# sail-sg/finetune-fair-diffusion

Measured on AMD Instinct MI355X. Metric: training-images/sec (SD-v1.5 512^2, 20-step DPM-Solver++ unroll, fairness-finetune step), higher is better.
Workload: dtype f16

## Files before the change

finetune_fair_diffusion_amd/csrc/gemm.hip:

```cpp
#include "gemm_device.h"

template <int BM, int BN, bool CONV>
__global__ __launch_bounds__(256) void gemm_glds_kernel(fd_gemm_desc p, int ntm, int ntn) {
    FD_WG_TRACE(1);
    constexpr int TM = BM / 32, TN = BN / 32;
    constexpr int AI = BM / 64, BI = BN / 64;
    constexpr int EPI_HALFS = 4 * (BM / 2) * (BN / 2 + 4);
    constexpr int OPS_HALFS = 2 * (BM + BN) * 32;
    __shared__ __attribute__((aligned(16))) f16 smem[OPS_HALFS > EPI_HALFS ? OPS_HALFS : EPI_HALFS];
    f16* As = smem;
    f16* Bs = smem + 2 * BM * 32;
    const f16* zp = fd_zero_page;
    asm volatile("" : "+s"(zp));

    const int tid = threadIdx.x, lane = tid & 63, wave = tid >> 6;
    const int l15 = lane & 15, lg = lane >> 4;
    const int wm = wave >> 1, wn = wave & 1;

    const int tile = xcd_remap(blockIdx.x, ntm * ntn);
    const int m0 = (tile / ntn) * BM, n0 = (tile % ntn) * BN;
    const int z = blockIdx.y;

    const f16* A = (const f16*)p.A + (int64_t)z * p.sA;
    const f16* B = (const f16*)p.B + (int64_t)z * p.sB;
// ... 448 lines not shown
    const int ntm = (d.M + BM - 1) / BM, ntn = (d.N + BN - 1) / BN;
    constexpr size_t lds = (size_t)2 * (BM + BN) * 64 * sizeof(f16);
    static std::once_flag once;
    std::call_once(once, [] {
        (void)hipFuncSetAttribute((const void*)gemm_big_kernel<BM, BN, WGM, WGN, 0>, hipFuncAttributeMaxDynamicSharedMemorySize, (int)lds);
        (void)hipFuncSetAttribute((const void*)gemm_big_kernel<BM, BN, WGM, WGN, 1>, hipFuncAttributeMaxDynamicSharedMemorySize, (int)lds);
        (void)hipFuncSetAttribute((const void*)gemm_big_kernel<BM, BN, WGM, WGN, 2>, hipFuncAttributeMaxDynamicSharedMemorySize, (int)lds);
    });
    static const long l2_budget = bench_env("FD_GEMM_L2_KB") ? atol(bench_env("FD_GEMM_L2_KB")) * 1024 : 3 * 1024 * 1024;
    const long ktot = ((long)d.K + d.K2) / nsplit;
    const int nph = (d.conv && (d.conv_mode == FD_CONV_UP2P || d.conv_mode == FD_CONV_UP2PI)) ? 4 : 1;
    long gnl = l2_budget / ((long)BN * ktot * 2);
    const int gn = (int)(gnl < 1 ? 1 : (gnl > ntn ? ntn : gnl));
    if constexpr (BN / WGN == 80) {
        if (d.gn_stats && nsplit == 1 && d.conv && d.conv_mode == FD_CONV_UP2PI) {
            static std::once_flag once_st6;
            std::call_once(once_st6, [] {
                (void)hipFuncSetAttribute((const void*)gemm_big_kernel<BM, BN, WGM, WGN, 6>, hipFuncAttributeMaxDynamicSharedMemorySize, (int)lds);
            });
            hipLaunchKernelGGL((gemm_big_kernel<BM, BN, WGM, WGN, 6>), dim3(ntm * ntn * nph, 1), dim3(WGM * WGN * 64), lds, s, d, ntm, ntn, gn);
            return fd_check_launch("fd_gemm(big, phase pair with statistics epilogue)");
        }
        if (d.gn_stats && nsplit == 1 && !(d.conv && d.conv_mode >= FD_CONV_UP2P)) {
            static std::once_flag once_st;
            std::call_once(once_st, [] {
                (void)hipFuncSetAttribute((const void*)gemm_big_kernel<BM, BN, WGM, WGN, 3>, hipFuncAttributeMaxDynamicSharedMemorySize, (int)lds);
                (void)hipFuncSetAttribute((const void*)gemm_big_kernel<BM, BN, WGM, WGN, 4>, hipFuncAttributeMaxDynamicSharedMemorySize, (int)lds);
            });
            if (d.conv) hipLaunchKernelGGL((gemm_big_kernel<BM, BN, WGM, WGN, 4>), dim3(ntm * ntn, 1), dim3(WGM * WGN * 64), lds, s, d, ntm, ntn, gn);
            else hipLaunchKernelGGL((gemm_big_kernel<BM, BN, WGM, WGN, 3>), dim3(ntm * ntn, 1), dim3(WGM * WGN * 64), lds, s, d, ntm, ntn, gn);
            return fd_check_launch("fd_gemm(big, statistics epilogue)");
        }
    }
    if (d.conv && d.conv_mode >= FD_CONV_UP2P)
        hipLaunchKernelGGL((gemm_big_kernel<BM, BN, WGM, WGN, 2>), dim3(ntm * ntn * nph, nsplit), dim3(WGM * WGN * 64), lds, s, d, ntm, ntn, gn);
    else if (d.conv) hipLaunchKernelGGL((gemm_big_kernel<BM, BN, WGM, WGN, 1>), dim3(ntm * ntn, nsplit), dim3(WGM * WGN * 64), lds, s, d, ntm, ntn, gn);
    else hipLaunchKernelGGL((gemm_big_kernel<BM, BN, WGM, WGN, 0>), dim3(ntm * ntn, nsplit), dim3(WGM * WGN * 64), lds, s, d, ntm, ntn, gn);
    if (nsplit > 1) return launch_splitk_reduce(d, s, nsplit);
    return fd_check_launch("fd_gemm(big)");
}


template <int NT, int KS, int RT>
__global__ __launch_bounds__(KS * 64) void gemm_skinny_kernel(fd_gemm_desc p) {
    FD_WG_TRACE(4);
    __shared__ float red[KS > 1 ? (KS - 1) * RT * NT * 256 : 1];
    const int lane = threadIdx.x & 63, wave = threadIdx.x >> 6;
    const int l15 = lane & 15, lg = lane >> 4;
    const f16* A[RT];
    bool mok[RT];
#pragma unroll
    for (int r = 0; r < RT; ++r) {
        const int m = (blockIdx.x * RT + r) * 16 + l15;
        mok[r] = m < p.M;
        A[r] = (const f16*)p.A + (int64_t)(mok[r] ? m : 0) * p.lda + lg * 8;
    }
    const f16* B = (const f16*)p.B + lg * 8;
    f32x4 acc[RT][NT];
#pragma unroll
    for (int r = 0; r < RT; ++r)
#pragma unroll
        for (int j = 0; j < NT; ++j) acc[r][j] = (f32x4){0.f, 0.f, 0.f, 0.f};
    const int nks = p.K >> 5;
    const int per = (nks + KS - 1) / KS;
    const int kbeg = wave * per, kend = min(nks, kbeg + per);
    constexpr int CH = 10 / RT;
    for (int k0 = kbeg; k0 < kend; k0 += CH) {
        f16x8 af[RT][CH];
#pragma unroll
        for (int c = 0; c < CH; ++c)
#pragma unroll
            for (int r = 0; r < RT; ++r) {
                af[r][c] = (f16x8){0, 0, 0, 0, 0, 0, 0, 0};
                if (k0 + c < kend && mok[r]) af[r][c] = *(const f16x8*)(A[r] + (int64_t)(k0 + c) * 32);
            }
#pragma unroll
        for (int c = 0; c < CH; ++c) {
            if (k0 + c < kend) {
#pragma unroll
                for (int j = 0; j < NT; ++j) {
                    const int n = j * 16 + l15;
                    f16x8 bf = (f16x8){0, 0, 0, 0, 0, 0, 0, 0};
                    if (n < p.N) bf = *(const f16x8*)(B + (int64_t)n * p.ldb + (int64_t)(k0 + c) * 32);
#pragma unroll
                    for (int r = 0; r < RT; ++r) acc[r][j] = FD_MFMA_16x16x32(bf, af[r][c], acc[r][j]);
                }
            }
        }
    }
    if (KS > 1) {
        if (wave > 0) {
#pragma unroll
            for (int r = 0; r < RT; ++r)
#pragma unroll
                for (int j = 0; j < NT; ++j) *(f32x4*)(red + ((((wave - 1) * RT + r) * NT + j) * 64 + lane) * 4) = acc[r][j];
        }
        __syncthreads();
        if (wave > 0) return;
#pragma unroll
        for (int w = 1; w < KS; ++w)
#pragma unroll
            for (int r = 0; r < RT; ++r)
#pragma unroll
                for (int j = 0; j < NT; ++j) acc[r][j] += *(const f32x4*)(red + ((((w - 1) * RT + r) * NT + j) * 64 + lane) * 4);
    }
#pragma unroll
    for (int r = 0; r < RT; ++r) {
        if (!mok[r]) continue;
        f16* C = (f16*)p.C + (int64_t)((blockIdx.x * RT + r) * 16 + l15) * p.ldc;
#pragma unroll
        for (int j = 0; j < NT; ++j) {
            const int n = j * 16 + lg * 4;
            if (n < p.N) *(f16x4*)(C + n) = (f16x4){(f16)acc[r][j][0], (f16)acc[r][j][1], (f16)acc[r][j][2], (f16)acc[r][j][3]};
        }
    }
}

static bool skinny_ok(const fd_gemm_desc& d) {
    static const bool off = bench_env("FD_GEMM_NOSKINNY") != nullptr;
    if (d.N > 16 && d.M >= 32768) return false;
    return !off && !d.conv && d.batch <= 1 && d.K2 == 0 && d.colscale_cols == 0 && d.N <= 64 && (d.N & 3) == 0 && (d.K & 31) == 0 && d.M >= 1024 && !d.bias && !d.rowbias &&
           !d.residual && d.act == FD_ACT_NONE && d.alpha == 1.f && d.out_dtype == FD_OUT_F16 && (d.ldc & 3) == 0;
}

template <int NT, int RT>
static int launch_skinny_rt(const fd_gemm_desc& d, hipStream_t s) {
    const int blocks = (d.M + 16 * RT - 1) / (16 * RT);
    const int ks = d.K >= 1280 ? 4 : d.K >= 640 ? 2 : 1;
    if (ks == 4) hipLaunchKernelGGL((gemm_skinny_kernel<NT, 4, RT>), dim3(blocks), dim3(256), 0, s, d);
    else if (ks == 2) hipLaunchKernelGGL((gemm_skinny_kernel<NT, 2, RT>), dim3(blocks), dim3(128), 0, s, d);
    else hipLaunchKernelGGL((gemm_skinny_kernel<NT, 1, RT>), dim3(blocks), dim3(64), 0, s, d);
    return fd_check_launch("fd_gemm(skinny)");
}

template <int NT>
static int launch_skinny(const fd_gemm_desc& d, hipStream_t s) {
    static const int rt = bench_env("FD_GEMM_SKINNY_RT") ? atoi(bench_env("FD_GEMM_SKINNY_RT")) : 0;
    const bool two = rt == 2;
    return two ? launch_skinny_rt<NT, 2>(d, s) : launch_skinny_rt<NT, 1>(d, s);
}

template <int BM, int BN>
static int launch(const fd_gemm_desc& d, hipStream_t s) {
    const int ntm = (d.M + BM - 1) / BM, ntn = (d.N + BN - 1) / BN;
    dim3 grid(ntm * ntn, d.batch > 0 ? d.batch : 1);
    if (d.conv) hipLaunchKernelGGL((gemm_glds_kernel<BM, BN, true>), grid, dim3(256), 0, s, d, ntm, ntn);
    else hipLaunchKernelGGL((gemm_glds_kernel<BM, BN, false>), grid, dim3(256), 0, s, d, ntm, ntn);
    return fd_check_launch("fd_gemm");
}

bool fd_gemm_pp_eligible(const fd_gemm_desc& d);
int fd_gemm_launch_pp(const fd_gemm_desc& d, hipStream_t s, bool prio, int bm, int nsplit);
bool fd_conv_halo_takes(const fd_gemm_desc& d, int bm, int nsplit);
#ifndef FD_GEMM_PP_DEFAULT
#define FD_GEMM_PP_DEFAULT (1 | 4 | 8 | 32)
#endif
static int pp_mode() {
#ifdef FD_BENCH_HOOKS
    const char* e = getenv("FD_GEMM_PP");
    return e ? atoi(e) : FD_GEMM_PP_DEFAULT;
#else
    return FD_GEMM_PP_DEFAULT;
#endif
}
static int pp_takes(const fd_gemm_desc& d, int sel) {
    const int t = sel % 1000000, split = sel / 1000000, m = pp_mode();
    if (!m || !fd_gemm_pp_eligible(d)) return 0;
    if (t == 256320 && split == 0) {
        if (d.conv) return (m & 1) ? 256 : 0;
        if ((m & 2) || ((m & 32) && d.K + d.K2 <= 384 && d.N >= 2560)) return 256;
        return 0;
    }
    if (t == 128320 && (split == 0 || (m & 64))) return (m & (d.conv ? 8 : 16)) ? 128 : 0;
    return 0;
}

static int gemm_tile(const fd_gemm_desc& d);
extern "C" int fd_gemm_tile(const fd_gemm_desc* dp) {
    FD_REQUIRE_DESC(dp, fd_gemm_desc, "fd_gemm_tile");
    return gemm_tile(*dp);
}
static int gemm_tile(const fd_gemm_desc& d) {
    const long nb = d.batch > 1 ? d.batch : 1;
    static const bool nobig = bench_env("FD_GEMM_NOBIG") != nullptr;
    static const int force = bench_env("FD_GEMM_FORCE") ? atoi(bench_env("FD_GEMM_FORCE")) : 0;
    if (skinny_ok(d)) return 16000 + (d.N + 15) / 16 * 16;
    if (force && nb == 1 && !d.conv) return force;
    static const int bigk = bench_env("FD_GEMM_BIGK") ? atoi(bench_env("FD_GEMM_BIGK")) : 320;
    if (!nobig && nb == 1 && (d.conv ? (d.Cin & 63) == 0 : (d.K + d.K2) >= bigk)) {
        const long phs = (d.conv && (d.conv_mode == FD_CONV_UP2P || d.conv_mode == FD_CONV_UP2PI)) ? 4 : 1;
        const long m256 = phs * ((d.M + 255) / 256), m128 = phs * ((d.M + 127) / 128);
        static const long t256 = bench_env("FD_GEMM_T256") ? atol(bench_env("FD_GEMM_T256")) : 100;
        static const long t128 = bench_env("FD_GEMM_T128") ? atol(bench_env("FD_GEMM_T128")) : 80;
        static const long maxsplit = bench_env("FD_GEMM_MAXSPLIT") ? atol(bench_env("FD_GEMM_MAXSPLIT")) : 8;
        static const long tc256 = bench_env("FD_CONV_T256") ? atol(bench_env("FD_CONV_T256")) : 0;
        if (d.N % 320 == 0) {
            if (m256 * (d.N / 320) >= ((tc256 && d.conv && d.conv_mode == FD_CONV_NORMAL) ? tc256 : t256)) return 256320;
            if (m128 * (d.N / 320) >= t128) return 128320;
        }
        const bool can_split = d.workspace && (d.N & 3) == 0 && (d.ldc & 3) == 0 && d.act != FD_ACT_GEGLU && phs == 1;
        const long nk = (d.K + 63) / 64 + (d.K2 + 63) / 64;
        auto split_for = [&](long blocks, int tilecode) -> int {
            long split = blocks > 0 ? 256 / blocks : 1;
            if (split > maxsplit) split = maxsplit;
            while (split > 1 && (nk / split < 8 || (int64_t)split * d.M * d.N * 4 > d.workspace_bytes)) --split;
            return split > 1 ? (int)(split * 1000000 + tilecode) : 0;
        };
        if (can_split && nk >= 64 && d.N % 320 == 0 && m128 * (d.N / 320) >= 32) {
            const int c = split_for(m128 * (d.N / 320), 128320);
            if (c) return c;
        }
        static const long t160 = bench_env("FD_GEMM_T160") ? atol(bench_env("FD_GEMM_T160")) : 160;
        if (d.N % 160 == 0 && m128 * (d.N / 160) >= t160) return 128160;
        static const bool no256 = bench_env("FD_GEMM_NO256256") != nullptr;
        static const long tvae = bench_env("FD_GEMM_TVAE") ? atol(bench_env("FD_GEMM_TVAE")) : 200;
        if (!no256 && d.N % 256 == 0 && m256 * (d.N / 256) >= tvae) return 256256;
        static const bool no512 = bench_env("FD_GEMM_NO512128") != nullptr;
        if (!no512 && d.N == 128 && ((d.M + 511) / 512) >= 400) return 512128;
        if (d.N % 128 == 0 && m256 * (d.N / 128) >= tvae) return 256128;
        if (can_split && d.N % 160 == 0) {
            const int c = split_for(m128 * (d.N / 160), 128160);
            if (c) return c;
        }
    }
    const long t128 = (long)((d.M + 127) / 128) * ((d.N + 127) / 128) * nb;
    const bool n64 = (d.N % 128) != 0 && (d.N % 128) <= 64;
    if (t128 >= 512 && !n64) return 128128;
    const long t12864 = (long)((d.M + 127) / 128) * ((d.N + 63) / 64) * nb;
    if (t12864 >= 512) return 128064;
    return 64064;
}

enum { GK_SKINNY, GK_GLDS, GK_BIG, GK_PP };
struct GemmPlan { int kind, bm, bn, wgm, wgn, nsplit, cv; bool stats_ok; };
static GemmPlan gemm_plan(const fd_gemm_desc& d ) {
    GemmPlan g = {};
    const int sel = gemm_tile(d), t = sel % 1000000;
    static const bool w16 = bench_env("FD_GEMM_W8") == nullptr;
    g.nsplit = sel >= 1000000 ? sel / 1000000 : 1;
    g.bm = t / 1000; g.bn = t % 1000;
    g.cv = d.conv ? (d.conv_mode >= FD_CONV_UP2P ? 2 : 1) : 0;
    if (const int bm = pp_takes(d, sel)) { g.kind = GK_PP; g.bm = bm; g.bn = 320; g.wgm = 2; g.wgn = 4; }
    else if (g.nsplit > 1) { g.kind = GK_BIG; g.wgm = 4; g.wgn = t == 128320 ? 4 : 2; }
    else switch (t) {
        case 256320: g.kind = GK_BIG; g.wgm = (w16 && !d.conv) ? 4 : 2; g.wgn = 4; break;
        case 128320: g.kind = GK_BIG; g.wgm = w16 ? 4 : 2; g.wgn = 4; break;
        case 128160: g.kind = GK_BIG; g.wgm = 4; g.wgn = 2; break;
        case 256256: g.kind = GK_BIG; g.wgm = 2; g.wgn = 4; break;
        case 512128: g.kind = GK_BIG; g.wgm = 8; g.wgn = 2; break;
        case 256128: g.kind = GK_BIG; g.wgm = 4; g.wgn = 2; break;
        default: g.kind = g.bm == 16 ? GK_SKINNY : GK_GLDS; break;
    }
    const bool lds_epi = d.out_dtype == FD_OUT_F16 && (d.N & 7) == 0 && (d.ldc & 7) == 0 && (!d.residual || (d.ldr & 7) == 0) &&
                         (!d.rowbias || (d.ld_rowbias & 3) == 0);
    g.stats_ok = (g.kind == GK_PP || (g.kind == GK_BIG && g.bn / g.wgn == 80)) && g.nsplit == 1 && lds_epi && d.act != FD_ACT_GEGLU &&
                 d.batch <= 1 && (d.N % 80) == 0 && (g.cv < 2 || (d.conv_mode == FD_CONV_UP2PI && (d.M & 31) == 0));
    return g;
}

extern "C" int fd_gemm_kernel_name(const fd_gemm_desc* dp, char* buf, int n) {
    FD_REQUIRE_DESC(dp, fd_gemm_desc, "fd_gemm_kernel_name");
    fd_gemm_desc d = *dp;
    if (d.K2 <= 0 || !d.A2) d.K2 = 0;
    const GemmPlan g = gemm_plan(d);
    const bool st = d.gn_stats && g.stats_ok;
    switch (g.kind) {
        case GK_PP:
            if (fd_conv_halo_takes(d, g.bm, g.nsplit)) snprintf(buf, n, "conv_halo_kernel<%d, %d, %d, %s>", g.bm, d.W, st ? 3 : 1, (pp_mode() & 4) ? "true" : "false");
            else snprintf(buf, n, "gemm_pp_kernel<%d, %d, %s>", g.bm, (d.conv ? 1 : 0) + (st ? 2 : 0), (pp_mode() & 4) ? "true" : "false");
            break;
        case GK_BIG: snprintf(buf, n, "gemm_big_kernel<%d, %d, %d, %d, %d>", g.bm, g.bn, g.wgm, g.wgn, st ? (g.cv == 2 ? 6 : g.cv + 3) : g.cv); break;
        case GK_SKINNY: snprintf(buf, n, "gemm_skinny_kernel<%d, %d, 1>", g.bn / 16, d.K >= 1280 ? 4 : d.K >= 640 ? 2 : 1); break;
        default: snprintf(buf, n, "gemm_glds_kernel<%d, %d, %s>", g.bm, g.bn, d.conv ? "true" : "false"); break;
    }
    return g.nsplit > 1 ? g.nsplit : 0;
}

extern "C" int fd_gemm_stats_rows(const fd_gemm_desc* dp) {
    FD_REQUIRE_DESC(dp, fd_gemm_desc, "fd_gemm_stats_rows");
    fd_gemm_desc d = *dp;
    if (d.K2 <= 0 || !d.A2) d.K2 = 0;
    return gemm_plan(d).stats_ok ? 32 : 0;
}

extern "C" int fd_gemm(const fd_gemm_desc* dp, void* stream) {
    FD_REQUIRE_DESC(dp, fd_gemm_desc, "fd_gemm");
    fd_gemm_desc d = *dp;
#ifdef FD_BENCH_HOOKS
    static const char* dbg = bench_env("FD_GEMM_DBG");
    if (dbg && d.batch <= 1) d.batch = -atoi(dbg);
#endif
    FD_REQUIRE(d.A && d.B && d.C, "fd_gemm: null operand");
    FD_REQUIRE(d.M > 0 && d.N > 0 && d.K > 0, "fd_gemm: bad shape M=%d N=%d K=%d", d.M, d.N, d.K);
    FD_REQUIRE((d.K & 7) == 0 && (d.lda & 7) == 0 && (d.ldb & 7) == 0, "fd_gemm: K, lda, ldb must be multiples of 8");
    if (d.K2 > 0) {
        FD_REQUIRE(!d.conv, "fd_gemm: second K-slab not supported with conv gather");
        FD_REQUIRE(d.A2 && d.B2 && (d.K2 & 7) == 0 && (d.lda2 & 7) == 0 && (d.ldb2 & 7) == 0, "fd_gemm: bad second slab");
        FD_REQUIRE(d.batch <= 1, "fd_gemm: second slab is not batched");
    } else d.K2 = 0;
    if (d.conv) {
        const bool up_fwd = d.conv_mode == FD_CONV_UP2P || d.conv_mode == FD_CONV_UP2PI;
        const int ntap = up_fwd ? 4 : d.conv_mode == FD_CONV_UP2P_BWD ? 16 : 9;
        FD_REQUIRE((d.Cin & 31) == 0 && d.K == ntap * d.Cin, "fd_gemm(conv): Cin must be a multiple of 32 and K == taps*Cin");
        if (up_fwd) FD_REQUIRE(!d.residual && !d.rowbias, "fd_gemm(conv up2 phases): bias-only epilogue");
        if (d.conv_mode == FD_CONV_UP2PI) FD_REQUIRE(d.out_dtype == FD_OUT_F16, "fd_gemm(conv up2 phases, interleaved result): fp16 output");
        FD_REQUIRE(d.M == d.Bn * d.Ho * d.Wo, "fd_gemm(conv): M != B*Ho*Wo");
        FD_REQUIRE(d.batch <= 1, "fd_gemm(conv): not batched");
        FD_REQUIRE((int64_t)d.Bn * d.H * d.W * d.lda < (1LL << 31), "fd_gemm(conv): input larger than 2^31 elements");
    }
    if (d.rowbias) FD_REQUIRE(d.rows_per_batch > 0, "fd_gemm: rows_per_batch");
    FD_REQUIRE(d.colscale_cols >= 0 && (d.colscale_cols & 3) == 0 && (d.colscale_cols == 0 || (d.act != FD_ACT_GEGLU && d.batch <= 1)),
               "fd_gemm: colscale_cols=%d must be a multiple of 4 (not with GEGLU / batched launches)", d.colscale_cols);
    if (d.act == FD_ACT_GEGLU)
        FD_REQUIRE(!d.conv && d.batch <= 1 && d.out_dtype == FD_OUT_F16 && !d.rowbias && d.alpha == 1.f && (d.N & 15) == 0 &&
                       (d.ldc & 7) == 0 && d.K2 == 0 && (!d.residual || (d.ldr & 7) == 0),
                   "fd_gemm(GEGLU): needs a plain fp16 GEMM with N %% 16 == 0 and ldc, ldr %% 8 == 0");
    hipStream_t s = (hipStream_t)stream;
    const GemmPlan g = gemm_plan(d);
    if (d.gn_stats) FD_REQUIRE(g.stats_ok, "fd_gemm: gn_stats set but the kernel for M=%d N=%d K=%d has no statistics epilogue (ask fd_gemm_stats_rows first)",
                               d.M, d.N, d.K);
    if (d.conv && d.conv_mode >= FD_CONV_UP2P)
        FD_REQUIRE(g.kind == GK_BIG, "fd_gemm(conv up2 phases): shape not taken by the big-tile kernels (Cin %% 64, enough tiles); use FD_CONV_UP2");
    switch (g.kind) {
        case GK_PP: {
            const int rc = fd_gemm_launch_pp(d, s, (pp_mode() & 4) != 0, g.bm, g.nsplit);
            if (rc != 0 || g.nsplit == 1) return rc;
            return launch_splitk_reduce(d, s, g.nsplit);
        }
        case GK_SKINNY:
            switch (g.bn) {
                case 16: return launch_skinny<1>(d, s);
                case 32: return launch_skinny<2>(d, s);
                case 48: return launch_skinny<3>(d, s);
                default: return launch_skinny<4>(d, s);
            }
        case GK_BIG:
            switch (g.bm * 1000 + g.bn) {
                case 256320: return g.wgm == 4 ? launch_big<256, 320, 4, 4>(d, s, g.nsplit) : launch_big<256, 320, 2, 4>(d, s, g.nsplit);
                case 128320: return g.wgm == 4 ? launch_big<128, 320, 4, 4>(d, s, g.nsplit) : launch_big<128, 320, 2, 4>(d, s, g.nsplit);
                case 128160: return launch_big<128, 160, 4, 2>(d, s, g.nsplit);
                case 256256: return launch_big<256, 256, 2, 4>(d, s, g.nsplit);
                case 512128: return launch_big<512, 128, 8, 2>(d, s, g.nsplit);
                default: return launch_big<256, 128, 4, 2>(d, s, g.nsplit);
            }
        default:
            if (g.bm == 128 && g.bn == 128) return launch<128, 128>(d, s);
            if (g.bm == 128 && g.bn == 64) return launch<128, 64>(d, s);
            return launch<64, 64>(d, s);
    }
}

FD_WGT_SETTER(gemm)
```

finetune_fair_diffusion_amd/csrc/gemm_halo.hip:

```cpp
#include "gemm_pp_device.h"

template <int BM, int W>
struct halo_geo {
    static constexpr int R = BM / W, S = W + 8;
    static constexpr int NPX = (R + 2) * S;
    static constexpr int NPIECE = NPX / 16;
    static constexpr int NAP = (NPIECE + PP_NW - 1) / PP_NW;
    static constexpr int ABUF = NPIECE * PP_GROUP;
    static_assert(BM % W == 0 && (BM / 2) % W == 0 && NPX % 16 == 0 && W % 16 == 0, "tile = whole image rows, wave tiles too");
};
constexpr int HALO_BST = PP_NGB * PP_GROUP;
template <int BM, int W> constexpr size_t halo_lds() { return (size_t)(2 * halo_geo<BM, W>::ABUF + PP_NST * HALO_BST + PP_NW * PP_GROUP) * sizeof(f16); }

#ifndef HALO_A_AUX
#define HALO_A_AUX 0
#endif
__device__ __forceinline__ int halo_swz(int P) { return ((P >> 2) & 1) << 1; }

template <int BM, int W, int CV, bool PRIO>
__global__ __launch_bounds__(512) void conv_halo_kernel(fd_gemm_desc p, int ntm, int ntn, int gn) {
    FD_WG_TRACE(6);
#if __HIP_DEVICE_COMPILE__
    using G = halo_geo<BM, W>;
    constexpr bool WSTATS = CV >= 2;
    constexpr int WTM = BM / 2, WTN = 80, TM = WTM / 16, TN = 5;
    constexpr int NAP = G::NAP, S = G::S;
    extern __shared__ __attribute__((aligned(16))) f16 smem[];
    const int tid = threadIdx.x, lane = tid & 63;
    const int wave = __builtin_amdgcn_readfirstlane(tid >> 6);
    const int l15 = lane & 15, lg = lane >> 4;
    const int wm = wave >> 2, wn = wave & 3;
    const bool lead = wave < 4;

    int tile = xcd_remap(blockIdx.x, gridDim.x);
    int mt, nt;
    if (gn >= ntn) {
        mt = tile / ntn;
        nt = tile - mt * ntn;
    } else {
        const int per = ntm * gn, nbands = (ntn + gn - 1) / gn;
        const int band = min(tile / per, nbands - 1);
        const int r = tile - band * per;
        const int w = band == nbands - 1 ? ntn - band * gn : gn;
        mt = r / w;
        nt = band * gn + (r - mt * w);
    }
    const int m0 = mt * BM, n0 = nt * PP_BN;
    const int img = m0 / (W * W), y0 = (m0 - img * W * W) / W;

    const int nch = p.Cin >> 5, nk = nch * 9;

    f16* const abuf = smem;
    f16* const ring = smem + 2 * G::ABUF;
    f16* const dump = ring + PP_NST * HALO_BST + wave * PP_GROUP;

    const __amdgpu_buffer_rsrc_t rA = __builtin_amdgcn_make_buffer_rsrc((void*)p.A, 0, (int)(uint32_t)((int64_t)p.Bn * W * W * p.lda * 2), 0x00020000);
    const __amdgpu_buffer_rsrc_t rB = __builtin_amdgcn_make_buffer_rsrc((void*)p.B, 0, (int)(uint32_t)((int64_t)p.N * p.ldb * 2), 0x00020000);
    uint32_t a_src[NAP];
#pragma unroll
    for (int i = 0; i < NAP; ++i) {
        const int j = wave + PP_NW * i;
        const int P = j * 16 + (lane >> 2);
        const int r = P / S, c = P - r * S;
        const int x = c - 1, y = y0 - 1 + r;
        const bool valid = j < G::NPIECE && x >= 0 && x < W && y >= 0 && y < W;
        a_src[i] = valid ? (uint32_t)((((int64_t)(img * W + y) * W + x) * p.lda + (((lane & 3) ^ halo_swz(P)) << 3)) * 2) : 0xFFFFFFF0u;
    }
    const uint32_t b_src = (uint32_t)((n0 + wave * 16 + (lane >> 2)) * (int)p.ldb + ((lane & 3) ^ swz_g(lane >> 4)) * 8) * 2;
    const uint32_t b_gstep = (uint32_t)(PP_NW * 16 * (int)p.ldb) * 2;

    auto issueB = [&](int cc, int tap, auto nl_c) {
        constexpr int NL = decltype(nl_c)::value;
        const bool live = cc < nch;
        f16* st = live ? ring + ((cc * 9 + tap) & 3) * HALO_BST + wave * PP_GROUP : dump;
        const int gstep = live ? PP_NW * PP_GROUP : 0;
        uint32_t kk = live ? (uint32_t)(tap * p.Cin + (cc << 5)) * 2 : 0u;
        asm volatile("" : "+s"(kk));
#pragma unroll
        for (int i = 0; i < NL; ++i)
            __builtin_amdgcn_raw_ptr_buffer_load_lds(rB, (__attribute__((address_space(3))) void*)(st + i * gstep), 16, b_src, kk + i * b_gstep, 0, 0);
    };
    auto issueA = [&](int cc, auto i_c) {
        constexpr int i = decltype(i_c)::value;
        const int j = wave + PP_NW * i;
        const bool live = cc < nch && j < G::NPIECE;
        uint32_t c32 = live ? (uint32_t)(cc << 6) : 0u;
        asm volatile("" : "+s"(c32));
        __builtin_amdgcn_raw_ptr_buffer_load_lds(rA, (__attribute__((address_space(3))) void*)(live ? abuf + (cc & 1) * G::ABUF + j * PP_GROUP : dump), 16, a_src[i], c32, 0, HALO_A_AUX);
    };

    f32x4 acc[TM][TN];
#pragma unroll
    for (int i = 0; i < TM; ++i)
#pragma unroll
        for (int j = 0; j < TN; ++j) acc[i][j] = (f32x4){0.f, 0.f, 0.f, 0.f};

    const uint32_t lds0 = (uint32_t)(uintptr_t)(__attribute__((address_space(3))) void*)smem;
    const int P0 = (wm * WTM / W) * S + l15;
    uint32_t a_base[3];
#pragma unroll
    for (int kx = 0; kx < 3; ++kx) a_base[kx] = lds0 + (uint32_t)((P0 + kx) * 32 + ((lg ^ halo_swz(P0 + kx)) << 3)) * 2;
    const uint32_t bfrag = (uint32_t)(l15 * 32 + ((lg ^ swz_g(l15 >> 2)) * 8)) * 2;
    const uint32_t b_frag = lds0 + (uint32_t)(2 * G::ABUF + (wn * (WTN / 16)) * PP_GROUP) * 2 + bfrag;
    constexpr uint32_t ABUF_B = G::ABUF * 2, BST_B = HALO_BST * 2, GROUP_B = PP_GROUP * 2;

    auto run = [&](auto nlb_c, auto lead_c) {
        constexpr int NLB = decltype(nlb_c)::value;
        constexpr bool LEAD = decltype(lead_c)::value;
        std::integral_constant<int, NLB> nl;
        static_for<0, NAP>([&](auto ic) { issueA(0, ic); });
        issueB(0, 0, nl); issueB(0, 1, nl); issueB(0, 2, nl);
        wait_vm<2 * NLB>();
        raw_barrier();
#pragma unroll 1
        for (int c = 0; c < nch; ++c) {
            const uint32_t ab = (uint32_t)(c & 1) * ABUF_B;
            static_for<0, 9>([&](auto tc) {
                constexpr int t = decltype(tc)::value;
                constexpr int ky = t / 3, kx = t % 3;
                constexpr int NW = NLB + ((((t + 8) % 9) < NAP) ? 1 : 0);
                constexpr int t3 = (t + 3) % 9;
                const int c3 = c + (t + 3) / 9;
                uint32_t so = (uint32_t)((c * 9 + t) & 3) * BST_B, ao = ab + (uint32_t)(ky * S * 64);
                asm volatile("" : "+s"(so), "+s"(ao));
                const uint32_t aa = a_base[kx] + ao;
                auto issue = [&] {
                    issueB(c3, t3, nl);
                    if constexpr (t < NAP) issueA(c + 1, tc);
#ifdef HALO_GN_PROBE
                    if constexpr (t >= 6) {
                        constexpr int NITEM = G::NPIECE * 64, PER = (NITEM + 511) / 512;
                        constexpr int J0 = t == 6 ? 0 : (t == 7 ? (PER + 2) / 3 : 2 * ((PER + 2) / 3)), J1 = t == 6 ? (PER + 2) / 3 : (t == 7 ? 2 * ((PER + 2) / 3) : PER);
                        f16* nb = abuf + ((c + 1) & 1) * G::ABUF;
                        const float* tab = (const float*)(ring + PP_NST * HALO_BST);
#pragma unroll
                        for (int j = J0; j < J1; ++j) {
                            const int it = min(tid + 512 * j, NITEM - 1);
                            {
                                f16x8 v = *(f16x8*)(nb + it * 8);
#pragma unroll
                                for (int h = 0; h < 2; ++h) {
                                    const f32x4 sc = *(const f32x4*)(tab + (it & 3) * 16 + h * 4), sh = *(const f32x4*)(tab + (it & 3) * 16 + 8 + h * 4);
#pragma unroll
                                    for (int e = 0; e < 4; ++e) v[h * 4 + e] = (f16)silu_f((float)v[h * 4 + e] * sc[e] + sh[e]);
                                    asm volatile("" : "+v"(v));
                                }
                                *(f16x8*)(nb + it * 8) = v;
                            }
                        }
                    }
#endif
                };
                if constexpr (LEAD) {
                    auto mid = [&] {
                        wait_vm<NW>();
                        raw_barrier();
                    };
                    mma_k32_mid<TM, TN, 2, GROUP_B, PRIO, decltype(mid)&, 0, W>(acc, aa, b_frag + so, mid);
                    issue();
                } else {
                    wait_vm<NW>();
                    raw_barrier();
                    issue();
                    auto mid = [] {};
                    mma_k32_mid<TM, TN, 2, GROUP_B, PRIO, decltype(mid)&, 0, W>(acc, aa, b_frag + so, mid);
                }
            });
        }
    };
    if (lead) run(std::integral_constant<int, 3>{}, std::true_type{});
    else run(std::integral_constant<int, 2>{}, std::false_type{});

    asm volatile("s_waitcnt vmcnt(0)" ::: "memory");
    __syncthreads();

    const bool lds_epi = p.out_dtype == FD_OUT_F16 && (p.N & 7) == 0 && (p.ldc & 7) == 0 && (!p.residual || (p.ldr & 7) == 0) &&
                         (!p.rowbias || (p.ld_rowbias & 3) == 0);
    constexpr int TMC = BM == 256 ? TM / 2 : TM;
    static_assert(PP_NW * TMC * 16 * (WTN + 4) <= 2 * G::ABUF + PP_NST * HALO_BST, "epilogue staging does not fit the operand area");
    if (lds_epi) {
        gemm_epilogue_lds<TM, TN, TMC, WSTATS>(p, acc, smem + wave * (TMC * 16) * (WTN + 4), m0 + wm * WTM, n0 + wn * WTN, lane, 0, 0);
    } else {
        gemm_epilogue<TM, TN>(p, acc, m0 + wm * WTM, n0 + wn * WTN, l15, lg, 0, 0);
    }
#endif
}

template <int BM, int W, int CV, bool PRIO>
static void launch_halo(const fd_gemm_desc& d, hipStream_t s, int ntm, int ntn, int gn) {
    static std::once_flag once;
    std::call_once(once, [] {
        (void)hipFuncSetAttribute((const void*)conv_halo_kernel<BM, W, CV, PRIO>, hipFuncAttributeMaxDynamicSharedMemorySize, (int)halo_lds<BM, W>());
    });
    constexpr size_t lds = halo_lds<BM, W>();
    hipLaunchKernelGGL((conv_halo_kernel<BM, W, CV, PRIO>), dim3(ntm * ntn), dim3(512), lds, s, d, ntm, ntn, gn);
}

template <int BM, int W>
static void launch_halo_w(const fd_gemm_desc& d, hipStream_t s, bool prio) {
    const int ntm = d.M / BM, ntn = d.N / PP_BN;
    const long l2_budget = 3 * 1024 * 1024;
    long gnl = l2_budget / ((long)PP_BN * d.K * 2);
    const int gn = (int)(gnl < 1 ? 1 : (gnl > ntn ? ntn : gnl));
    (void)prio;
    if (d.gn_stats) launch_halo<BM, W, 3, true>(d, s, ntm, ntn, gn);
    else launch_halo<BM, W, 1, true>(d, s, ntm, ntn, gn);
}

bool fd_conv_halo_eligible(const fd_gemm_desc& d, int bm) {
    if (!d.conv || d.conv_mode != FD_CONV_NORMAL || d.batch > 1 || (d.N % 320) != 0 || (d.Cin & 31) != 0 || d.K2 != 0 || d.act == FD_ACT_GEGLU) return false;
    if (d.H != d.W || d.Ho != d.H || d.Wo != d.W || (d.W != 16 && d.W != 32 && d.W != 64)) return false;
    return (d.W * d.W) % bm == 0 && d.M % bm == 0 && (bm / 2) % d.W == 0 && (int64_t)d.N * d.ldb < (1LL << 31);
}

int fd_conv_halo_launch(const fd_gemm_desc& d, hipStream_t s, bool prio, int bm) {
#ifdef HALO_QUICK
    launch_halo<HALO_QUICK, 64, 1, true>(d, s, 1, 1, 1);
    return 0;
#else
    if (bm == 256) {
        if (d.W == 64) launch_halo_w<256, 64>(d, s, prio);
        else if (d.W == 32) launch_halo_w<256, 32>(d, s, prio);
        else launch_halo_w<256, 16>(d, s, prio);
    } else {
        if (d.W == 64) launch_halo_w<128, 64>(d, s, prio);
        else if (d.W == 32) launch_halo_w<128, 32>(d, s, prio);
        else launch_halo_w<128, 16>(d, s, prio);
    }
    return fd_check_launch("fd_gemm(conv halo)");
#endif
}

FD_WGT_SETTER(gemm_halo)
```

finetune_fair_diffusion_amd/csrc/gemm_pp.hip:

```cpp
#include "gemm_pp_device.h"

constexpr uint32_t PP_OOR = 0xFFFFFFF0u;
template <int BM, int CV, bool PRIO>
__global__ __launch_bounds__(512) void gemm_pp_kernel(fd_gemm_desc p, int ntm, int ntn, int gn) {
    FD_WG_TRACE(5);
    constexpr int CONV = CV & 1;
    constexpr bool WSTATS = CV >= 2;
    constexpr int WTM = BM / 2, WTN = 80, TM = WTM / 16, TN = 5;
    constexpr int NGA = BM / 16, NAW = NGA / PP_NW;
    constexpr int STAGE = pp_stage<BM>();
    extern __shared__ __attribute__((aligned(16))) f16 smem[];
    const f16* zp = fd_zero_page;
    asm volatile("" : "+s"(zp));

    const int tid = threadIdx.x, lane = tid & 63;
    const int wave = __builtin_amdgcn_readfirstlane(tid >> 6);
    const int l15 = lane & 15, lg = lane >> 4;
    const int wm = wave >> 2, wn = wave & 3;
    const bool lead = wave < 4;

    int tile = xcd_remap(blockIdx.x, gridDim.x);
    int mt, nt;
    if (gn >= ntn) {
        mt = tile / ntn;
// ... 107 lines not shown
            const uint32_t so = (uint32_t)k0 * 2;
            if (!seg2) {
#pragma unroll
                for (int i = 0; i < NAW; ++i)
                    __builtin_amdgcn_raw_ptr_buffer_load_lds(rA, (__attribute__((address_space(3))) void*)(st + (wave + 8 * i) * PP_GROUP), 16, kok ? a_vo[i] : PP_OOR, so, 0, 0);
#pragma unroll
                for (int i = 0; i < NL - NAW; ++i)
                    __builtin_amdgcn_raw_ptr_buffer_load_lds(rB, (__attribute__((address_space(3))) void*)(st + (NGA + wave + 8 * i) * PP_GROUP), 16, kok ? b_vo[i] : PP_OOR, so, 0, 0);
            } else {
#pragma unroll
                for (int i = 0; i < NAW; ++i)
                    __builtin_amdgcn_raw_ptr_buffer_load_lds(rA2, (__attribute__((address_space(3))) void*)(st + (wave + 8 * i) * PP_GROUP), 16, kok ? a_vo2[i] : PP_OOR, so, 0, 0);
#pragma unroll
                for (int i = 0; i < NL - NAW; ++i)
                    __builtin_amdgcn_raw_ptr_buffer_load_lds(rB2, (__attribute__((address_space(3))) void*)(st + (NGA + wave + 8 * i) * PP_GROUP), 16, kok ? b_vo2[i] : PP_OOR, so, 0, 0);
            }
#endif
        }
    };

    f32x4 acc[TM][TN];
#pragma unroll
    for (int i = 0; i < TM; ++i)
#pragma unroll
        for (int j = 0; j < TN; ++j) acc[i][j] = (f32x4){0.f, 0.f, 0.f, 0.f};

    const uint32_t lds0 = (uint32_t)(uintptr_t)(__attribute__((address_space(3))) void*)smem;
    const uint32_t frag = (uint32_t)(l15 * 32 + ((lg ^ swz_g(l15 >> 2)) * 8)) * 2;
    const uint32_t a_frag = lds0 + (uint32_t)(wm * (WTM / 16) * PP_GROUP) * 2 + frag;
    const uint32_t b_frag = lds0 + (uint32_t)((NGA + wn * (WTN / 16)) * PP_GROUP) * 2 + frag;
    constexpr uint32_t STAGE_B = STAGE * 2, GROUP_B = PP_GROUP * 2;

    auto main_loop = [&](auto abl_c, auto nosync_c) {
        constexpr int ABL = decltype(abl_c)::value;
        constexpr bool NOSYNC = decltype(nosync_c)::value;
        if (lead) {
            constexpr int NL = NAW + 3;
            std::integral_constant<int, NL> nl;
            issue(0, nl); issue(1, nl); issue(2, nl);
            wait_vm<2 * NL>();
            raw_barrier();
            for (int i = 0; i < nk; ++i) {
                const uint32_t so = (uint32_t)(i & 3) * STAGE_B;
                auto mid = [&] {
                    if (!NOSYNC) {
                        wait_vm<NL>();
                        raw_barrier();
                    }
                };
                mma_k32_mid<TM, TN, 2, GROUP_B, PRIO, decltype(mid)&, ABL>(acc, a_frag + so, b_frag + so, mid);
                issue(i + 3, nl);
            }
        } else {
            constexpr int NL = NAW + 2;
            std::integral_constant<int, NL> nl;
            issue(0, nl); issue(1, nl); issue(2, nl);
            wait_vm<2 * NL>();
            raw_barrier();
            for (int i = 0; i < nk; ++i) {
                if (!NOSYNC) {
                    wait_vm<NL>();
                    raw_barrier();
                }
                issue(i + 3, nl);
                const uint32_t so = (uint32_t)(i & 3) * STAGE_B;
                auto mid = [] {};
                mma_k32_mid<TM, TN, 2, GROUP_B, PRIO, decltype(mid)&, ABL>(acc, a_frag + so, b_frag + so, mid);
            }
        }
    };
#ifdef FD_BENCH_HOOKS
    if (FD_DBG_IS(p, 2)) main_loop(std::integral_constant<int, 2>{}, std::false_type{});
    else if (FD_DBG_IS(p, 6)) main_loop(std::integral_constant<int, 6>{}, std::false_type{});
    else if (FD_DBG_IS(p, 7)) main_loop(std::integral_constant<int, 0>{}, std::true_type{});
    else
#endif
    main_loop(std::integral_constant<int, 0>{}, std::false_type{});
    if (nsplit > 1) {
        float* ws = (float*)p.workspace + (int64_t)blockIdx.y * p.M * p.N;
#pragma unroll
        for (int i = 0; i < TM; ++i) {
            const int m = m0 + wm * WTM + i * 16 + l15;
            if (m >= p.M) continue;
#pragma unroll
            for (int j = 0; j < TN; ++j) {
                const int n = n0 + wn * WTN + j * 16 + lg * 4;
                if (n < p.N) *(f32x4*)(ws + (int64_t)m * p.N + n) = acc[i][j];
            }
        }
        return;
    }
    asm volatile("s_waitcnt vmcnt(0)" ::: "memory");
    __syncthreads();
    if (FD_DBG_IS(p, 3)) {
        if (acc[0][0][0] == 12345.678f) ((f16*)p.C)[0] = (f16)1.f;
        return;
    }

    const bool lds_epi = p.out_dtype == FD_OUT_F16 && (p.N & 7) == 0 && (p.ldc & 7) == 0 && (!p.residual || (p.ldr & 7) == 0) &&
                         (!p.rowbias || (p.ld_rowbias & 3) == 0);
    constexpr int TMC = BM == 256 ? TM / 2 : TM;
    static_assert(PP_NW * TMC * 16 * (WTN + 4) <= PP_NST * STAGE, "epilogue staging does not fit the ring");
    if (p.act == FD_ACT_GEGLU) {
        gemm_epilogue_geglu_lds<TM, TN, TMC>(p, acc, smem + wave * (TMC * 16) * (WTN + 4), m0 + wm * WTM, n0 + wn * WTN, lane);
    } else if (lds_epi) {
        gemm_epilogue_lds<TM, TN, TMC, WSTATS>(p, acc, smem + wave * (TMC * 16) * (WTN + 4), m0 + wm * WTM, n0 + wn * WTN, lane, 0, 0);
    } else {
        gemm_epilogue<TM, TN>(p, acc, m0 + wm * WTM, n0 + wn * WTN, l15, lg, 0, 0);
    }
}

template <int BM, int CV, bool PRIO>
static void launch_pp(const fd_gemm_desc& d, hipStream_t s, int ntm, int ntn, int gn, int nsplit) {
    static std::once_flag once;
    std::call_once(once, [] {
        (void)hipFuncSetAttribute((const void*)gemm_pp_kernel<BM, CV, PRIO>, hipFuncAttributeMaxDynamicSharedMemorySize, (int)pp_lds<BM>());
    });
    hipLaunchKernelGGL((gemm_pp_kernel<BM, CV, PRIO>), dim3(ntm * ntn, nsplit), dim3(512), pp_lds<BM>(), s, d, ntm, ntn, gn);
}

template <int BM>
static void launch_pp_bm(const fd_gemm_desc& d, hipStream_t s, bool prio, int nsplit) {
    const int ntm = (d.M + BM - 1) / BM, ntn = d.N / PP_BN;
    const long l2_budget = 3 * 1024 * 1024;
    const long ktot = ((long)d.K + d.K2) / nsplit;
    long gnl = l2_budget / ((long)PP_BN * ktot * 2);
    const int gn = (int)(gnl < 1 ? 1 : (gnl > ntn ? ntn : gnl));
    if (d.gn_stats && nsplit == 1) {
        if (d.conv) { if (prio) launch_pp<BM, 3, true>(d, s, ntm, ntn, gn, 1); else launch_pp<BM, 3, false>(d, s, ntm, ntn, gn, 1); }
        else { if (prio) launch_pp<BM, 2, true>(d, s, ntm, ntn, gn, 1); else launch_pp<BM, 2, false>(d, s, ntm, ntn, gn, 1); }
        return;
    }
    if (d.conv) { if (prio) launch_pp<BM, 1, true>(d, s, ntm, ntn, gn, nsplit); else launch_pp<BM, 1, false>(d, s, ntm, ntn, gn, nsplit); }
    else { if (prio) launch_pp<BM, 0, true>(d, s, ntm, ntn, gn, nsplit); else launch_pp<BM, 0, false>(d, s, ntm, ntn, gn, nsplit); }
}

bool fd_gemm_pp_eligible(const fd_gemm_desc& d) {
    if (d.batch > 1 || (d.N % 320) != 0) return false;
    if (d.conv) return d.conv_mode == FD_CONV_NORMAL && (d.Cin & 31) == 0 && d.K2 == 0;
    const int64_t lim = 1LL << 31;
    return (d.K & 7) == 0 && (int64_t)d.M * d.lda < lim && (int64_t)d.N * d.ldb < lim && (d.K2 == 0 || ((int64_t)d.M * d.lda2 < lim && (int64_t)d.N * d.ldb2 < lim));
}

bool fd_conv_halo_eligible(const fd_gemm_desc& d, int bm);
int fd_conv_halo_launch(const fd_gemm_desc& d, hipStream_t s, bool prio, int bm);
bool fd_conv_halo_takes(const fd_gemm_desc& d, int bm, int nsplit) {
#ifdef FD_BENCH_HOOKS
    const char* e = getenv("FD_CONV_HALO");
    if (e && atoi(e) == 0) return false;
#endif
    return nsplit == 1 && fd_conv_halo_eligible(d, bm);
}

int fd_gemm_launch_pp(const fd_gemm_desc& d, hipStream_t s, bool prio, int bm, int nsplit) {
    if (fd_conv_halo_takes(d, bm, nsplit)) return fd_conv_halo_launch(d, s, prio, bm);
    if (bm == 256) launch_pp_bm<256>(d, s, prio, nsplit);
    else launch_pp_bm<128>(d, s, prio, nsplit);
    return fd_check_launch("fd_gemm(pp)");
}

FD_WGT_SETTER(gemm_pp)
```

Measured before the change: 6.249.

## Extend halo-conv kernel to wide VAE convolutions with row-segment tiles

Generalizes the halo-staged 3x3 conv kernel so one tile can cover a horizontal segment of an image row (X pixels) rather than whole rows. Output tiles can now also be 128 or 256 wide, with the wave grid and B-load split derived from the tile shape. A new GK_HALOW plan routes the large-resolution convs (W=64 or W a multiple of 128, such as in the VAE) that previously went to gemm_big_kernel with implicit im2col into this kernel. The aim is to reuse each loaded input halo across all 9 taps from LDS instead of re-gathering for every tap. The cost is more template instantiations and tighter LDS and geometry constraints, which static asserts enforce.

Measured after the change: 6.248. Within noise of the previous version (-0.0%).

```diff
diff --git a/finetune_fair_diffusion_amd/csrc/gemm.hip b/finetune_fair_diffusion_amd/csrc/gemm.hip
--- a/finetune_fair_diffusion_amd/csrc/gemm.hip
+++ b/finetune_fair_diffusion_amd/csrc/gemm.hip
@@ -624,6 +624,8 @@
 bool fd_gemm_pp_eligible(const fd_gemm_desc& d);
 int fd_gemm_launch_pp(const fd_gemm_desc& d, hipStream_t s, bool prio, int bm, int nsplit);
 bool fd_conv_halo_takes(const fd_gemm_desc& d, int bm, int nsplit);
+int fd_conv_halo_wide_takes(const fd_gemm_desc& d, int tile, int nsplit);
+int fd_conv_halo_wide_launch(const fd_gemm_desc& d, hipStream_t s, int code);
 #ifndef FD_GEMM_PP_DEFAULT
 #define FD_GEMM_PP_DEFAULT (1 | 4 | 8 | 32)
 #endif
@@ -703,8 +705,8 @@
     return 64064;
 }
 
-enum { GK_SKINNY, GK_GLDS, GK_BIG, GK_PP };
-struct GemmPlan { int kind, bm, bn, wgm, wgn, nsplit, cv; bool stats_ok; };
+enum { GK_SKINNY, GK_GLDS, GK_BIG, GK_PP, GK_HALOW };
+struct GemmPlan { int kind, bm, bn, wgm, wgn, nsplit, cv, halow; bool stats_ok; };
 static GemmPlan gemm_plan(const fd_gemm_desc& d ) {
     GemmPlan g = {};
     const int sel = gemm_tile(d), t = sel % 1000000;
@@ -713,6 +715,9 @@
     g.bm = t / 1000; g.bn = t % 1000;
     g.cv = d.conv ? (d.conv_mode >= FD_CONV_UP2P ? 2 : 1) : 0;
     if (const int bm = pp_takes(d, sel)) { g.kind = GK_PP; g.bm = bm; g.bn = 320; g.wgm = 2; g.wgn = 4; }
+    else if ((g.halow = fd_conv_halo_wide_takes(d, t, g.nsplit)) != 0) {
+        g.kind = GK_HALOW; g.bm = g.halow / 1000000; g.bn = g.halow % 1000; g.wgn = g.bn / 64; g.wgm = 8 / g.wgn;
+    }
     else if (g.nsplit > 1) { g.kind = GK_BIG; g.wgm = 4; g.wgn = t == 128320 ? 4 : 2; }
     else switch (t) {
         case 256320: g.kind = GK_BIG; g.wgm = (w16 && !d.conv) ? 4 : 2; g.wgn = 4; break;
@@ -741,6 +746,7 @@
             if (fd_conv_halo_takes(d, g.bm, g.nsplit)) snprintf(buf, n, "conv_halo_kernel<%d, %d, %d, %s>", g.bm, d.W, st ? 3 : 1, (pp_mode() & 4) ? "true" : "false");
             else snprintf(buf, n, "gemm_pp_kernel<%d, %d, %s>", g.bm, (d.conv ? 1 : 0) + (st ? 2 : 0), (pp_mode() & 4) ? "true" : "false");
             break;
+        case GK_HALOW: snprintf(buf, n, "conv_halo_wide_kernel<%d, %d, %d>", g.bm, g.halow / 1000 % 1000, g.bn); break;
         case GK_BIG: snprintf(buf, n, "gemm_big_kernel<%d, %d, %d, %d, %d>", g.bm, g.bn, g.wgm, g.wgn, st ? (g.cv == 2 ? 6 : g.cv + 3) : g.cv); break;
         case GK_SKINNY: snprintf(buf, n, "gemm_skinny_kernel<%d, %d, 1>", g.bn / 16, d.K >= 1280 ? 4 : d.K >= 640 ? 2 : 1); break;
         default: snprintf(buf, n, "gemm_glds_kernel<%d, %d, %s>", g.bm, g.bn, d.conv ? "true" : "false"); break;
@@ -799,6 +805,7 @@
             if (rc != 0 || g.nsplit == 1) return rc;
             return launch_splitk_reduce(d, s, g.nsplit);
         }
+        case GK_HALOW: return fd_conv_halo_wide_launch(d, s, g.halow);
         case GK_SKINNY:
             switch (g.bn) {
                 case 16: return launch_skinny<1>(d, s);
diff --git a/finetune_fair_diffusion_amd/csrc/gemm_halo.hip b/finetune_fair_diffusion_amd/csrc/gemm_halo.hip
--- a/finetune_fair_diffusion_amd/csrc/gemm_halo.hip
+++ b/finetune_fair_diffusion_amd/csrc/gemm_halo.hip
@@ -1,35 +1,44 @@
 #include "gemm_pp_device.h"
 
-template <int BM, int W>
+template <int BM, int X, int BN>
 struct halo_geo {
-    static constexpr int R = BM / W, S = W + 8;
+    static constexpr int R = BM / X, S = X + 8;
     static constexpr int NPX = (R + 2) * S;
-    static constexpr int NPIECE = NPX / 16;
+    static constexpr int NPIECE = (NPX + 15) / 16;
     static constexpr int NAP = (NPIECE + PP_NW - 1) / PP_NW;
     static constexpr int ABUF = NPIECE * PP_GROUP;
-    static_assert(BM % W == 0 && (BM / 2) % W == 0 && NPX % 16 == 0 && W % 16 == 0, "tile = whole image rows, wave tiles too");
+    static constexpr int WGN = BN == 320 ? 4 : BN / 64, WGM = PP_NW / WGN;
+    static constexpr int WTM = BM / WGM, WTN = BN / WGN;
+    static constexpr int NGB = BN / 16;
+    static constexpr int NLB_LEAD = (NGB + PP_NW - 1) / PP_NW, NLB_REST = NGB / PP_NW;
+    static constexpr int BST = NGB * PP_GROUP;
+    static constexpr size_t LDS = (size_t)(2 * ABUF + PP_NST * BST + PP_NW * PP_GROUP) * sizeof(f16);
+    static_assert(BM % X == 0 && X % 16 == 0 && S % 8 == 0, "tile = whole rows of the segment; the row stride keeps (P >> 2) & 1 of a column");
+    static_assert(WTM % X == 0 || X % WTM == 0, "a wave tile is whole segment rows or an aligned part of one");
+    static_assert(NAP <= 7, "the A pieces of the next chunk ride with taps 0 .. NAP - 1 and the last one must land before tap 8's barrier");
+    static_assert(NGB % 4 == 0 && (NGB % PP_NW == 0 || NGB % PP_NW == 4) && WTM % 16 == 0 && WTN % 16 == 0, "B groups per wave");
+    static_assert(LDS <= 160 * 1024, "two A buffers + the B ring + the dump groups fit the LDS");
 };
-constexpr int HALO_BST = PP_NGB * PP_GROUP;
-template <int BM, int W> constexpr size_t halo_lds() { return (size_t)(2 * halo_geo<BM, W>::ABUF + PP_NST * HALO_BST + PP_NW * PP_GROUP) * sizeof(f16); }
 
 #ifndef HALO_A_AUX
 #define HALO_A_AUX 0
 #endif
 __device__ __forceinline__ int halo_swz(int P) { return ((P >> 2) & 1) << 1; }
 
-template <int BM, int W, int CV, bool PRIO>
-__global__ __launch_bounds__(512) void conv_halo_kernel(fd_gemm_desc p, int ntm, int ntn, int gn) {
-    FD_WG_TRACE(6);
 #if __HIP_DEVICE_COMPILE__
-    using G = halo_geo<BM, W>;
+template <int BM, int X, int BN, int CV, bool PRIO, bool FULL>
+__device__ __forceinline__ void halo_tile(const fd_gemm_desc& p, int ntm, int ntn, int gn) {
+    using G = halo_geo<BM, X, BN>;
     constexpr bool WSTATS = CV >= 2;
-    constexpr int WTM = BM / 2, WTN = 80, TM = WTM / 16, TN = 5;
-    constexpr int NAP = G::NAP, S = G::S;
+    constexpr int WTM = G::WTM, WTN = G::WTN, TM = WTM / 16, TN = WTN / 16;
+    constexpr int NAP = G::NAP, S = G::S, R = G::R;
+    constexpr int HALO_BST = G::BST;
+    static_assert(FULL || WTM <= X, "the rows of a wave tile are consecutive rows of C");
     extern __shared__ __attribute__((aligned(16))) f16 smem[];
     const int tid = threadIdx.x, lane = tid & 63;
     const int wave = __builtin_amdgcn_readfirstlane(tid >> 6);
     const int l15 = lane & 15, lg = lane >> 4;
-    const int wm = wave >> 2, wn = wave & 3;
+    const int wm = wave / G::WGN, wn = wave % G::WGN;
     const bool lead = wave < 4;
 
     int tile = xcd_remap(blockIdx.x, gridDim.x);
@@ -45,8 +54,11 @@
         mt = r / w;
         nt = band * gn + (r - mt * w);
     }
-    const int m0 = mt * BM, n0 = nt * PP_BN;
-    const int img = m0 / (W * W), y0 = (m0 - img * W * W) / W;
+    const int n0 = nt * BN;
+    const int W = FULL ? X : p.W, H = FULL ? X : p.H;
+    const int nsx = W / X, nsy = H / R;
+    const int xs = mt % nsx, ys = (mt / nsx) % nsy, img = mt / (nsx * nsy);
+    const int x0 = xs * X, y0 = ys * R;
 
     const int nch = p.Cin >> 5, nk = nch * 9;
 
@@ -54,7 +66,7 @@
     f16* const ring = smem + 2 * G::ABUF;
     f16* const dump = ring + PP_NST * HALO_BST + wave * PP_GROUP;
 
-    const __amdgpu_buffer_rsrc_t rA = __builtin_amdgcn_make_buffer_rsrc((void*)p.A, 0, (int)(uint32_t)((int64_t)p.Bn * W * W * p.lda * 2), 0x00020000);
+    const __amdgpu_buffer_rsrc_t rA = __builtin_amdgcn_make_buffer_rsrc((void*)p.A, 0, (int)(uint32_t)((int64_t)p.Bn * H * W * p.lda * 2), 0x00020000);
     const __amdgpu_buffer_rsrc_t rB = __builtin_amdgcn_make_buffer_rsrc((void*)p.B, 0, (int)(uint32_t)((int64_t)p.N * p.ldb * 2), 0x00020000);
     uint32_t a_src[NAP];
 #pragma unroll
@@ -62,9 +74,9 @@
         const int j = wave + PP_NW * i;
         const int P = j * 16 + (lane >> 2);
         const int r = P / S, c = P - r * S;
-        const int x = c - 1, y = y0 - 1 + r;
-        const bool valid = j < G::NPIECE && x >= 0 && x < W && y >= 0 && y < W;
-        a_src[i] = valid ? (uint32_t)((((int64_t)(img * W + y) * W + x) * p.lda + (((lane & 3) ^ halo_swz(P)) << 3)) * 2) : 0xFFFFFFF0u;
+        const int x = x0 + c - 1, y = y0 - 1 + r;
+        const bool valid = j < G::NPIECE && c < X + 2 && r < R + 2 && x >= 0 && x < W && y >= 0 && y < H;
+        a_src[i] = valid ? (uint32_t)((((int64_t)(img * H + y) * W + x) * p.lda + (((lane & 3) ^ halo_swz(P)) << 3)) * 2) : 0xFFFFFFF0u;
     }
     const uint32_t b_src = (uint32_t)((n0 + wave * 16 + (lane >> 2)) * (int)p.ldb + ((lane & 3) ^ swz_g(lane >> 4)) * 8) * 2;
     const uint32_t b_gstep = (uint32_t)(PP_NW * 16 * (int)p.ldb) * 2;
@@ -96,7 +108,7 @@
         for (int j = 0; j < TN; ++j) acc[i][j] = (f32x4){0.f, 0.f, 0.f, 0.f};
 
     const uint32_t lds0 = (uint32_t)(uintptr_t)(__attribute__((address_space(3))) void*)smem;
-    const int P0 = (wm * WTM / W) * S + l15;
+    const int P0 = (wm * WTM / X) * S + (wm * WTM) % X + l15;
     uint32_t a_base[3];
 #pragma unroll
     for (int kx = 0; kx < 3; ++kx) a_base[kx] = lds0 + (uint32_t)((P0 + kx) * 32 + ((lg ^ halo_swz(P0 + kx)) << 3)) * 2;
@@ -156,33 +168,50 @@
                         wait_vm<NW>();
                         raw_barrier();
                     };
-                    mma_k32_mid<TM, TN, 2, GROUP_B, PRIO, decltype(mid)&, 0, W>(acc, aa, b_frag + so, mid);
+                    mma_k32_mid<TM, TN, 2, GROUP_B, PRIO, decltype(mid)&, 0, X>(acc, aa, b_frag + so, mid);
                     issue();
                 } else {
                     wait_vm<NW>();
                     raw_barrier();
                     issue();
                     auto mid = [] {};
-                    mma_k32_mid<TM, TN, 2, GROUP_B, PRIO, decltype(mid)&, 0, W>(acc, aa, b_frag + so, mid);
+                    mma_k32_mid<TM, TN, 2, GROUP_B, PRIO, decltype(mid)&, 0, X>(acc, aa, b_frag + so, mid);
                 }
             });
         }
     };
-    if (lead) run(std::integral_constant<int, 3>{}, std::true_type{});
-    else run(std::integral_constant<int, 2>{}, std::false_type{});
+    if (lead) run(std::integral_constant<int, G::NLB_LEAD>{}, std::true_type{});
+    else run(std::integral_constant<int, G::NLB_REST>{}, std::false_type{});
 
     asm volatile("s_waitcnt vmcnt(0)" ::: "memory");
     __syncthreads();
 
     const bool lds_epi = p.out_dtype == FD_OUT_F16 && (p.N & 7) == 0 && (p.ldc & 7) == 0 && (!p.residual || (p.ldr & 7) == 0) &&
                          (!p.rowbias || (p.ld_rowbias & 3) == 0);
-    constexpr int TMC = BM == 256 ? TM / 2 : TM;
+    constexpr int TMC = TM == 8 ? TM / 2 : TM;
     static_assert(PP_NW * TMC * 16 * (WTN + 4) <= 2 * G::ABUF + PP_NST * HALO_BST, "epilogue staging does not fit the operand area");
+    const int mw = (img * H + y0 + wm * WTM / X) * W + x0 + (wm * WTM) % X;
     if (lds_epi) {
-        gemm_epilogue_lds<TM, TN, TMC, WSTATS>(p, acc, smem + wave * (TMC * 16) * (WTN + 4), m0 + wm * WTM, n0 + wn * WTN, lane, 0, 0);
+        gemm_epilogue_lds<TM, TN, TMC, WSTATS>(p, acc, smem + wave * (TMC * 16) * (WTN + 4), mw, n0 + wn * WTN, lane, 0, 0);
     } else {
-        gemm_epilogue<TM, TN>(p, acc, m0 + wm * WTM, n0 + wn * WTN, l15, lg, 0, 0);
-    }
+        gemm_epilogue<TM, TN>(p, acc, mw, n0 + wn * WTN, l15, lg, 0, 0);
+    }
+}
+#endif
+
+template <int BM, int W, int CV, bool PRIO>
+__global__ __launch_bounds__(512) void conv_halo_kernel(fd_gemm_desc p, int ntm, int ntn, int gn) {
+    FD_WG_TRACE(6);
+#if __HIP_DEVICE_COMPILE__
+    halo_tile<BM, W, PP_BN, CV, PRIO, true>(p, ntm, ntn, gn);
+#endif
+}
+
+template <int BM, int X, int BN>
+__global__ __launch_bounds__(512) void conv_halo_wide_kernel(fd_gemm_desc p, int ntm, int ntn, int gn) {
+    FD_WG_TRACE(6);
+#if __HIP_DEVICE_COMPILE__
+    halo_tile<BM, X, BN, 1, true, (X < 128)>(p, ntm, ntn, gn);
 #endif
 }
 
@@ -190,9 +219,9 @@
 static void launch_halo(const fd_gemm_desc& d, hipStream_t s, int ntm, int ntn, int gn) {
     static std::once_flag once;
     std::call_once(once, [] {
-        (void)hipFuncSetAttribute((const void*)conv_halo_kernel<BM, W, CV, PRIO>, hipFuncAttributeMaxDynamicSharedMemorySize, (int)halo_lds<BM, W>());
+        (void)hipFuncSetAttribute((const void*)conv_halo_kernel<BM, W, CV, PRIO>, hipFuncAttributeMaxDynamicSharedMemorySize, (int)halo_geo<BM, W, PP_BN>::LDS);
     });
-    constexpr size_t lds = halo_lds<BM, W>();
+    constexpr size_t lds = halo_geo<BM, W, PP_BN>::LDS;
     hipLaunchKernelGGL((conv_halo_kernel<BM, W, CV, PRIO>), dim3(ntm * ntn), dim3(512), lds, s, d, ntm, ntn, gn);
 }
 
@@ -207,10 +236,48 @@
     else launch_halo<BM, W, 1, true>(d, s, ntm, ntn, gn);
 }
 
+template <int BM, int X, int BN>
+static void launch_halo_wide(const fd_gemm_desc& d, hipStream_t s) {
+    using G = halo_geo<BM, X, BN>;
+    static std::once_flag once;
+    std::call_once(once, [] { (void)hipFuncSetAttribute((const void*)conv_halo_wide_kernel<BM, X, BN>, hipFuncAttributeMaxDynamicSharedMemorySize, (int)G::LDS); });
+    const int ntm = d.M / BM, ntn = d.N / BN;
+    const long gnl = 3L * 1024 * 1024 / ((long)BN * d.K * 2);
+    const int gn = (int)(gnl < 1 ? 1 : (gnl > ntn ? ntn : gnl));
+    hipLaunchKernelGGL((conv_halo_wide_kernel<BM, X, BN>), dim3(ntm * ntn), dim3(512), G::LDS, s, d, ntm, ntn, gn);
+}
+
+static bool halo_operands_fit(const fd_gemm_desc& d) {
+    return (int64_t)d.Bn * d.H * d.W * d.lda < (1LL << 31) && ((int64_t)d.Bn * d.H * d.W * d.lda + d.Cin) * 2 + 16 < 0xFFFFFFF0LL && (int64_t)d.N * d.ldb < (1LL << 31);
+}
+static bool halo_conv_shape(const fd_gemm_desc& d) {
+    return d.conv && d.conv_mode == FD_CONV_NORMAL && d.batch <= 1 && (d.Cin & 31) == 0 && d.K2 == 0 && d.act != FD_ACT_GEGLU && d.H == d.W && d.Ho == d.H && d.Wo == d.W &&
+           d.M == d.Bn * d.H * d.W;
+}
+
 bool fd_conv_halo_eligible(const fd_gemm_desc& d, int bm) {
-    if (!d.conv || d.conv_mode != FD_CONV_NORMAL || d.batch > 1 || (d.N % 320) != 0 || (d.Cin & 31) != 0 || d.K2 != 0 || d.act == FD_ACT_GEGLU) return false;
-    if (d.H != d.W || d.Ho != d.H || d.Wo != d.W || (d.W != 16 && d.W != 32 && d.W != 64)) return false;
-    return (d.W * d.W) % bm == 0 && d.M % bm == 0 && (bm / 2) % d.W == 0 && (int64_t)d.N * d.ldb < (1LL << 31);
+    if (!halo_conv_shape(d) || (d.N % 320) != 0 || (d.W != 16 && d.W != 32 && d.W != 64)) return false;
+    return (d.W * d.W) % bm == 0 && d.M % bm == 0 && (bm / 2) % d.W == 0 && halo_operands_fit(d);
+}
+
+int fd_conv_halo_wide_code(const fd_gemm_desc& d, int tile) {
+    if (!halo_conv_shape(d) || !halo_operands_fit(d)) return 0;
+    if (tile == 256256 && d.N % 256 == 0) {
+        if (d.W == 64) return 256064256;
+        if (d.W % 128 == 0) return 256128256;
+    }
+    if ((tile == 512128 || tile == 256128) && d.N % 128 == 0 && d.W % 128 == 0 && (long)(d.M / 512) * (d.N / 128) >= 200) return 512128128;
+    return 0;
+}
+
+int fd_conv_halo_wide_launch(const fd_gemm_desc& d, hipStream_t s, int code) {
+    switch (code) {
+        case 256064256: launch_halo_wide<256, 64, 256>(d, s); break;
+        case 256128256: launch_halo_wide<256, 128, 256>(d, s); break;
+        case 512128128: launch_halo_wide<512, 128, 128>(d, s); break;
+        default: FD_REQUIRE(false, "fd_gemm(conv halo wide): no instantiation %d", code);
+    }
+    return fd_check_launch("fd_gemm(conv halo wide)");
 }
 
 int fd_conv_halo_launch(const fd_gemm_desc& d, hipStream_t s, bool prio, int bm) {
diff --git a/finetune_fair_diffusion_amd/csrc/gemm_pp.hip b/finetune_fair_diffusion_amd/csrc/gemm_pp.hip
--- a/finetune_fair_diffusion_amd/csrc/gemm_pp.hip
+++ b/finetune_fair_diffusion_amd/csrc/gemm_pp.hip
@@ -283,6 +283,23 @@
     return nsplit == 1 && fd_conv_halo_eligible(d, bm);
 }
 
+int fd_conv_halo_wide_code(const fd_gemm_desc& d, int tile);
+int fd_conv_halo_wide_takes(const fd_gemm_desc& d, int tile, int nsplit) {
+#ifdef FD_BENCH_HOOKS
+    const char* e = getenv("FD_CONV_HALO");
+    if (e && atoi(e) <= 1) return 0;
+#endif
+    const int code = nsplit == 1 ? fd_conv_halo_wide_code(d, tile) : 0;
+#ifdef FD_BENCH_HOOKS
+    const char* m = getenv("FD_CONV_HALO_WIDE");
+    if (m && code) {
+        const int bit = code == 256064256 ? 1 : code == 256128256 ? 2 : 4;
+        if (!(atoi(m) & bit)) return 0;
+    }
+#endif
+    return code;
+}
+
 int fd_gemm_launch_pp(const fd_gemm_desc& d, hipStream_t s, bool prio, int bm, int nsplit) {
     if (fd_conv_halo_takes(d, bm, nsplit)) return fd_conv_halo_launch(d, s, prio, bm);
     if (bm == 256) launch_pp_bm<256>(d, s, prio, nsplit);
```
